# callmeray/PointMVSNet

Hardware: AMD Instinct MI355X
Metric: depth-maps/sec (DTU 640x512, 3 src views, 2 flow iters) (higher is better)
Workload: dtype f32

## Files before the change

include/pointflow_hip.h:

```cpp
#ifndef POINTFLOW_HIP_H_
#define POINTFLOW_HIP_H_

#include <stdint.h>

#ifdef __cplusplus
extern "C" {
#endif

#define PF_OK 0
#define PF_ERR_INVALID_ARG (-1)
#define PF_ERR_UNSUPPORTED (-2)

#define PF_STATUS_BAD_INDEX 1u

#define PF_MAX_VIEWS 8
#define PF_GEMM_TILE 64

#define PF_CAM_KREF_INV 0
#define PF_CAM_RREF_INV 9
#define PF_CAM_TREF 18
#define PF_CAM_MEAN 21
#define PF_CAM_STD 24
#define PF_CAM_VIEWS 27
#define PF_CAM_VIEW_STRIDE 21
// ... 60 lines not shown
typedef struct pf_bn_job {
  const double* partials;
  int32_t T, pcols, col0, C;
  double count, unbias_n;
  const float* gamma;
  const float* beta;
  float* running_mean;
  float* running_var;
  float momentum, eps;
  int32_t G, groups_per_stat;
  float* scale;
  float* shift;
  int32_t ld_affine;
  int32_t rows4;
} pf_bn_job;
int pf_bn_finalize_jobs_f32(const pf_bn_job* jobs, int njobs, void* stream);


int pf_pointwise_gemm_f32(const float* X, int x_point_major, int64_t ldx, const float* Wt, float* Y,
                          int64_t ldy, int G, int Ng, int K, int Nc, int Nc_store, const float* in_scale,
                          const float* in_shift, const pf_bn_job* in_bn, int groups_per_stat, double* col_partials,
                          void* stream);

int pf_edge_stats_f32(const float* LE, int64_t ldle, int C, const int64_t* idx, int k, int G, int Ng,
                      double* partials, const uint8_t* codes, int lat_ks, int lat_h, int lat_w, void* stream);


int pf_edge_apply_f32(const float* LE, int64_t ldle, int C, const int64_t* idx, int k, int G, int Ng,
                      const float* scale, const float* shift, int ld_affine, int groups_per_stat,
                      int concat, float* Y, int64_t ldy, const uint8_t* codes, int lat_ks, int lat_h, int lat_w,
                      void* stream);

int pf_edge_backward_reduce_f32(const float* LE, int64_t ldle, int C, const int64_t* idx, int k, int G, int Ng,
                                const float* grad_y, int64_t ldg, const float* scale, const float* shift,
                                const float* mean, const float* invstd, int ld_affine, int groups_per_stat,
                                int concat, double* partials, void* stream);
int pf_edge_backward_apply_f32(const float* LE, int64_t ldle, int C, const int64_t* idx, int k, int G, int Ng,
                               const float* grad_y, int64_t ldg, const float* scale, const float* shift,
                               const float* mean, const float* invstd, const float* c1, const float* c2,
                               int ld_affine, int groups_per_stat, int concat, float* grad_le,
                               const uint32_t* inv_order, const uint32_t* inv_start, void* stream);

int pf_edge_backward_sums_f32(const float* LE, int64_t ldle, int C, const int64_t* idx, int k, int G, int Ng,
                              const float* grad_y, int64_t ldg, const float* scale, const float* shift,
                              const float* mean, const float* invstd, int ld_affine, int groups_per_stat, int concat,
                              double* partials, float* grad_le, float* grad_acc, int64_t ld_acc, int plane,
                              void* stream);
int pf_edge_backward_finish_f32(const float* LE, int64_t ldle, int C, int k, int G, int Ng, const float* grad_y,
                                int64_t ldg, const float* scale, const float* shift, const float* mean,
                                const float* invstd, const float* c1, const float* c2, int ld_affine,
                                int groups_per_stat, int concat, float* grad_le, const uint32_t* inv_order,
                                const uint32_t* inv_start, int plane, void* stream);

int pf_edge_backward_coeffs_f32(const double* partials, int G, int T, int cbn, int C, int concat, int groups_per_stat,
// ... 234 lines not shown
```

pointmvsnet_amd/_lib.py:

```python
import ctypes
import os

import torch

_HERE = os.path.dirname(os.path.abspath(__file__))
LIB_PATH = os.environ.get("PF_LIB_PATH") or os.path.join(_HERE, "libpointflow_hip.so")

_vp, _i, _i64, _f, _d = ctypes.c_void_p, ctypes.c_int, ctypes.c_int64, ctypes.c_float, ctypes.c_double



class BnJob(ctypes.Structure):
    _fields_ = [("partials", _vp), ("T", ctypes.c_int32), ("pcols", ctypes.c_int32), ("col0", ctypes.c_int32),
                ("C", ctypes.c_int32), ("count", _d), ("unbias_n", _d), ("gamma", _vp), ("beta", _vp),
                ("running_mean", _vp), ("running_var", _vp), ("momentum", _f), ("eps", _f),
                ("G", ctypes.c_int32), ("groups_per_stat", ctypes.c_int32), ("scale", _vp), ("shift", _vp),
                ("ld_affine", ctypes.c_int32), ("rows4", ctypes.c_int32)]


class WgradItem(ctypes.Structure):
    _fields_ = [("gr", _vp), ("x", _vp)] + [(n, _i64) for n in ("N", "Cg", "Cx", "Do", "Ho", "Wo", "Di", "Hi", "Wi")] + \
               [(n, ctypes.c_int32) for n in ("KD", "KH", "KW", "stride", "pd", "ph", "pw", "x_samples_per_stat")] + \
               [("x_scale", _vp), ("x_shift", _vp), ("workspace", _vp), ("workspace_bytes", _i64)] + \
               [(n, _i64) for n in ("rows_P", "ldg", "ldx", "x_rows_per_stat")]
# ... 34 lines not shown
    "pf_deconv3d_k3s2_f32": ([_vp, _vp, _vp, _vp, _i64, _i64, _i64, _i64, _i64, _i64, _vp, _vp, ctypes.POINTER(BnJob), _i,
                              _vp, _vp], _i),
    "pf_conv3d_bottom_supported": ([_i64, _i64, _i], _i),
    "pf_conv3d_bottom_blocks": ([_i64, _i64, _i64, _i], _i),
    "pf_conv3d_bottom_f32": ([_vp, _vp, _vp, _i64, _i64, _i64, _i64, _i64, _i64, _i, _vp, _vp, ctypes.POINTER(BnJob), _i,
                              _vp, _vp], _i),
    "pf_deconv3d_bottom_supported": ([_i64, _i64], _i),
    "pf_deconv3d_bottom_blocks": ([_i64, _i64, _i64], _i),
    "pf_deconv3d_bottom_f32": ([_vp, _vp, _vp, _i64, _i64, _i64, _i64, _i64, _i64, _vp, _vp, ctypes.POINTER(BnJob), _i,
                                _vp, _vp], _i),
    "pf_conv2d_wide_supported": ([_i64, _i64, _i, _i], _i),
    "pf_conv2d_wide_blocks": ([_i64, _i64, _i64, _i], _i),
    "pf_conv2d_wide_f32": ([_vp, _vp, _vp, _i64, _i64, _i64, _i64, _i64, _i, _i, _vp, _vp, ctypes.POINTER(BnJob), _i,
                            _vp, _i, _vp], _i),
    "pf_conv2d_wide_sets_f32": ([_vp, _i, _vp, _i64, _i, _vp, _i64, _i64, _i64, _i64, _i64, _i, _i, _vp, _vp,
                                 ctypes.POINTER(BnJob), _i, _vp, _i, _vp], _i),
    "pf_norm_blocks": ([_i64], _i),
    "pf_channel_stats_f32": ([_vp, _i64, _i64, _i64, _vp, _vp], _i),
    "pf_channel_affine_f32": ([_vp, _vp, _vp, _vp, _i64, _i64, _i64, _i, _i, _vp], _i),
    "pf_channel_bn_apply_f32": ([_vp, _vp, _vp, _i, _i64, _i64, _i64, _i, _d, _vp, _vp, _vp, _vp, _f, _f, _i, _vp, _vp], _i),
    "pf_channel_bn_apply2_f32": ([_vp, _vp, _i, _vp, _vp, _vp, _vp, _f, _f, _vp, _vp, _i, _vp, _vp, _vp, _vp, _f, _f, _vp,
                                  _i64, _i64, _i64, _i, _d, _vp], _i),
    "pf_channel_bn_fused_f32": ([_vp, _vp, _i64, _i64, _i64, _i, _vp, _vp, _vp, _vp, _f, _f, _i, _vp, _vp, _i, _vp], _i),
    "pf_edge_stats_f32": ([_vp, _i64, _i, _vp, _i, _i, _i, _vp, _vp, _i, _i, _i, _vp], _i),
    "pf_edge_backward_reduce_f32": ([_vp, _i64, _i, _vp, _i, _i, _i, _vp, _i64, _vp, _vp, _vp, _vp, _i, _i, _i, _vp, _vp], _i),
    "pf_edge_backward_apply_f32": ([_vp, _i64, _i, _vp, _i, _i, _i, _vp, _i64, _vp, _vp, _vp, _vp, _vp, _vp, _i, _i, _i,
                                    _vp, _vp, _vp, _vp], _i),
    "pf_edge_backward_sums_f32": ([_vp, _i64, _i, _vp, _i, _i, _i, _vp, _i64, _vp, _vp, _vp, _vp, _i, _i, _i, _vp, _vp, _vp,
                                   _i64, _i, _vp], _i),
    "pf_edge_backward_finish_f32": ([_vp, _i64, _i, _i, _i, _i, _vp, _i64, _vp, _vp, _vp, _vp, _vp, _vp, _i, _i, _i,
                                     _vp, _vp, _vp, _i, _vp], _i),
    "pf_knn_inverse_workspace": ([_i, _i, _i], _i64),
    "pf_knn_inverse": ([_vp, _i, _i, _i, _vp, _vp, _vp, _i64, _vp], _i),
    "pf_bn_finalize_f32": ([_vp, _i, _i, _i, _i, _d, _d, _vp, _vp, _vp, _vp, _f, _f, _i, _i, _vp, _vp, _i, _vp], _i),
    "pf_bn_finalize_jobs_f32": ([ctypes.POINTER(BnJob), _i, _vp], _i),
    "pf_edge_apply_f32": ([_vp, _i64, _i, _vp, _i, _i, _i, _vp, _vp, _i, _i, _i, _vp, _i64, _vp, _i, _i, _i, _vp], _i),
    "pf_flow_head_f32": ([_vp, _i64, _vp, _vp, _i, ctypes.POINTER(BnJob), _vp, _vp, _i, _i, _vp, _i, _i, _i, _vp, _vp,
                          _vp], _i),
    "pf_eval_pack_map_f32": ([_vp, _vp, _i, _i, _i, _vp], _i),
    "pf_eval_flow_prob_f32": ([_vp, _vp, _i, _i, _i, _vp], _i),
    "pf_eval_prob_filter_f32": ([_vp, _vp, _vp, _i, _i, _i, _i, _f, _f, _vp, _i, _vp], _i),
    "pf_fuse_stage_a_f32": ([_vp, _vp, _vp, _vp, _i, _i, _i, _f, _f, _f, _vp, _vp, _vp, _vp, _vp], _i),
    "pf_fuse_mark": ([_vp, _vp, _vp, _vp, _i, _i, _i, _i, _i, _vp], _i),
    "pf_fuse_compact_f32": ([_vp, _vp, _vp, _vp, _i64, _i64, _vp, _vp, _vp], _i),
    "pf_geo_filter_f32": ([_vp, _vp, _vp, _vp, _i, _i, _i, _i, _f, _f, _i, _f, _f, _vp, _vp, _vp, _vp, _vp], _i),
    "pf_cloud_cell_keys_f32": ([_vp, _i64, _f, _f, _f, _f, _i, _i, _i, _vp, _vp], _i),
    "pf_cloud_pack_f32": ([_vp, _vp, _i64, _i, _vp, _vp], _i),
    "pf_cloud_thin_round": ([_vp, _vp, _i64, _i, _i, _i, _f, _vp, _vp, _vp, _vp], _i),
    "pf_cloud_nn_cells_f32": ([_vp, _i64, _vp, _vp, _i64, _f, _f, _f, _f, _i, _i, _i, _i, _f, _vp, _vp, _vp, _vp], _i),
    "pf_cloud_nn_wave_f32": ([_vp, _vp, _i64, _i64, _vp, _vp, _i64, _f, _f, _f, _f, _i, _i, _i, _f, _vp, _vp, _vp], _i),
    "pf_cloud_obs_mask_f32": ([_vp, _i64, _vp, _i, _i, _i, _f, _f, _f, _f, _vp, _vp], _i),
    "pf_cloud_above_plane_f32": ([_vp, _i64, _f, _f, _f, _f, _vp, _vp], _i),
    "pf_preprocess_resize_u8": ([_vp, _i, _i, _i, _vp, _vp, _vp, _vp, _i, _i, _i, _vp, _vp, _vp], _i),
    "pf_preprocess_standardise_f32": ([_vp, _vp, _i, _i, _i, _vp, _vp], _i),
    "pf_scan_filter_supported": ([_i] * 7, _i),
    "pf_scan_filter_f32": ([_vp, _vp, _vp, _i, _i, _vp, _i, _i, _i, _i, _i, _i] + [_vp] * 8 + [_f, _f, _vp, _vp, _vp, _vp, _vp], _i),
    "pf_softargmin_prob_f32": ([_vp, _vp, _vp, _vp, _i64, _i64, _i64, _vp], _i),
    "pf_bn_train_rows_f32": ([_vp, _i, _i, _i, _i, _d, _d, _vp, _vp, _vp, _vp, _f, _f, _i, _i, _vp, _i, _i, _i, _vp], _i),
    "pf_bn_bwd_reduce_f32": ([_vp, _vp, _vp, _i64, _i64, _i64, _i, _i, _vp, _vp], _i),
# ... 176 lines not shown
```

pointmvsnet_amd/csrc/edgeconv.hip:

```cpp
#include <stdlib.h>

#include "pf_common.h"
#include "pf_bn_resolve.h"

namespace {

typedef float f32x16 __attribute__((ext_vector_type(16)));

constexpr int TILE = PF_GEMM_TILE;

constexpr int GT = 128;
constexpr int LDA = GT + 2;

template <bool POINT_MAJOR, int NT>
__global__ __launch_bounds__(256, 2) void pointwise_gemm_kernel(
    const float* __restrict__ X, int64_t ldx, const float* __restrict__ Wt, float* __restrict__ Y, int64_t ldy,
    int Ng, int K, int Nc_store, const float* __restrict__ in_scale, const float* __restrict__ in_shift,
    int groups_per_stat, double* __restrict__ partials, int T) {
  constexpr int NC = NT * 32;
  constexpr int KC = NT == 4 ? 16 : 32;
  constexpr int NA = KC * GT / 256;
  constexpr int NW = KC * NC / 256;
  __shared__ __attribute__((aligned(16))) float As[2][KC][LDA];
  __shared__ __attribute__((aligned(16))) float Ws[2][KC][NC];
// ... 378 lines not shown
      const int pd = c / k2, rem = c - pd * k2, ph = rem / lat.ks, pw = rem - ph * lat.ks;
      off = (pd - hk) * lat.H * lat.W + (ph - hk) * lat.W + (pw - hk);
    }
    lut[c] = off;
  }
  __syncthreads();
}

template <int C>
__device__ __forceinline__ void gather_rows_codes(const float* __restrict__ LE, int64_t ldle,
                                                  const uint8_t* __restrict__ cp, const int* lut, int64_t gbase, int n,
                                                  int Ng, int q, float4 (&e)[16]) {
  const uint4 cw = *reinterpret_cast<const uint4*>(cp);
  const unsigned w[4] = {cw.x, cw.y, cw.z, cw.w};
#pragma unroll
  for (int j = 0; j < 16; ++j) {
    const int code = (int)((w[j >> 2] >> (8 * (j & 3))) & 255u);
    int i = n + lut[code];
    i = i < 0 ? 0 : (i > Ng - 1 ? Ng - 1 : i);
    e[j] = ld4(LE + (gbase + i) * ldle + C + 4 * q);
  }
}

template <int C, int K>
__global__ __launch_bounds__(256) void edge_stats_kernel(const float* __restrict__ LE, int64_t ldle,
                                                         const int64_t* __restrict__ idx, int k, int Ng,
                                                         double* __restrict__ partials, int T,
                                                         unsigned* __restrict__ status,
                                                         const uint8_t* __restrict__ codes, Lattice lat) {
  constexpr int Q = C / 4;
  constexpr int PPB = 256 / Q;
  __shared__ double red[256 * 8];
  __shared__ int lut[256];
  if (K == 16 && codes != nullptr) build_code_lut(lut, lat);
  const int tid = threadIdx.x;
  const int q = tid % Q, pl = tid / Q;
  const int g = blockIdx.y, tb = blockIdx.x;
  const int tiles = (Ng + TILE - 1) / TILE;
  const int64_t gbase = (int64_t)g * Ng;
  double ds[4] = {0, 0, 0, 0}, dq[4] = {0, 0, 0, 0};
  bool bad = false;
  const int tile0 = xcd_tile(tb, lat);
  for (int tile = tile0; tile < tiles; tile += T) {
    const int n0 = tile * TILE;
    for (int p = pl; p < TILE; p += PPB) {
      const int n = n0 + p;
      if (n >= Ng) break;
      const int64_t row = gbase + n;
      const float4 l = ld4(LE + row * ldle + 4 * q);
      const int64_t* ip = idx + row * k;
      float4 s = {0, 0, 0, 0}, s2 = {0, 0, 0, 0};
      if constexpr (K > 0) {
        float4 e[K > 0 ? K : 1];
        if constexpr (K == 16) {
          if (codes != nullptr) gather_rows_codes<C>(LE, ldle, codes + row * 16, lut, gbase, n, Ng, q, e);
          else gather_rows<C, 16>(LE, ldle, ip, gbase, Ng, q, e, bad);
// ... 17 lines not shown
          const float dx = e.x - l.x, dy = e.y - l.y, dz = e.z - l.z, dw = e.w - l.w;
          s.x += dx; s.y += dy; s.z += dz; s.w += dw;
          s2.x += dx * dx; s2.y += dy * dy; s2.z += dz * dz; s2.w += dw * dw;
        }
      }
      ds[0] += (double)s.x; ds[1] += (double)s.y; ds[2] += (double)s.z; ds[3] += (double)s.w;
      dq[0] += (double)s2.x; dq[1] += (double)s2.y; dq[2] += (double)s2.z; dq[3] += (double)s2.w;
    }
  }
  if (bad) atomicOr(status, PF_STATUS_BAD_INDEX);
#pragma unroll
  for (int c = 0; c < 4; ++c) {
    red[tid * 8 + c] = ds[c];
    red[tid * 8 + 4 + c] = dq[c];
  }
  __syncthreads();
  if (tid < 2 * C) {
    const int qq = tid / 8, comp = tid % 8;
    double acc = 0.0;
    for (int s = 0; s < PPB; ++s) acc += red[(s * Q + qq) * 8 + comp];
    double* o = partials + (((int64_t)g * T + tile0) * C + 4 * qq + (comp & 3)) * 2 + (comp >> 2);
    *o = acc;
  }
}

template <int C, int K>
__global__ __launch_bounds__(256) void edge_apply_kernel(const float* __restrict__ LE, int64_t ldle,
                                                         const int64_t* __restrict__ idx, int k, int Ng,
                                                         const float* __restrict__ scale,
                                                         const float* __restrict__ shift, int ld_affine,
                                                         int groups_per_stat, int concat, float* __restrict__ Y,
                                                         int64_t ldy, int T, const uint8_t* __restrict__ codes,
                                                         Lattice lat) {
  constexpr int Q = C / 4;
  constexpr int PPB = 256 / Q;
  __shared__ int lut[256];
  if (K == 16 && codes != nullptr) build_code_lut(lut, lat);
  const int tid = threadIdx.x;
  const int q = tid % Q, pl = tid / Q;
  const int g = blockIdx.y, tb = blockIdx.x;
  const int tiles = (Ng + TILE - 1) / TILE;
  const int64_t gbase = (int64_t)g * Ng;
  const int64_t so = (int64_t)(g / groups_per_stat) * ld_affine;
  const int doff = concat ? C : 0;
  const float4 dsc = ld4(scale + so + doff + 4 * q), dsh = ld4(shift + so + doff + 4 * q);
  float4 csc = {0, 0, 0, 0}, csh = {0, 0, 0, 0};
  if (concat) {
    csc = ld4(scale + so + 4 * q);
    csh = ld4(shift + so + 4 * q);
  }
  const float kf = (float)k;
  bool bad = false;
  for (int tile = xcd_tile(tb, lat); tile < tiles; tile += T) {
    const int n0 = tile * TILE;
    for (int p = pl; p < TILE; p += PPB) {
      const int n = n0 + p;
      if (n >= Ng) break;
      const int64_t row = gbase + n;
      const float4 l = ld4(LE + row * ldle + 4 * q);
      const int64_t* ip = idx + row * k;
      float4 a = {0, 0, 0, 0};
      if constexpr (K > 0) {
        float4 e[K > 0 ? K : 1];
        if constexpr (K == 16) {
          if (codes != nullptr) gather_rows_codes<C>(LE, ldle, codes + row * 16, lut, gbase, n, Ng, q, e);
          else gather_rows<C, 16>(LE, ldle, ip, gbase, Ng, q, e, bad);
        } else {
          gather_rows<C, (K > 0 ? K : 2)>(LE, ldle, ip, gbase, Ng, q, e, bad);
        }
#pragma unroll
        for (int j = 0; j < K; ++j) {
          a.x += fmaxf(fmaf(e[j].x - l.x, dsc.x, dsh.x), 0.0f);
          a.y += fmaxf(fmaf(e[j].y - l.y, dsc.y, dsh.y), 0.0f);
          a.z += fmaxf(fmaf(e[j].z - l.z, dsc.z, dsh.z), 0.0f);
          a.w += fmaxf(fmaf(e[j].w - l.w, dsc.w, dsh.w), 0.0f);
        }
      } else {
        for (int j = 0; j < k; ++j) {
          int64_t i = ip[j];
          i = i < 0 ? 0 : (i >= Ng ? Ng - 1 : i);
          const float4 e = ld4(LE + (gbase + i) * ldle + C + 4 * q);
          a.x += fmaxf(fmaf(e.x - l.x, dsc.x, dsh.x), 0.0f);
          a.y += fmaxf(fmaf(e.y - l.y, dsc.y, dsh.y), 0.0f);
          a.z += fmaxf(fmaf(e.z - l.z, dsc.z, dsh.z), 0.0f);
          a.w += fmaxf(fmaf(e.w - l.w, dsc.w, dsh.w), 0.0f);
        }
      }
      float4 yd = {a.x / kf, a.y / kf, a.z / kf, a.w / kf};
      float* yo = Y + row * ldy + 4 * q;
      if (concat) {
        float4 yc = {fmaxf(fmaf(l.x, csc.x, csh.x), 0.0f), fmaxf(fmaf(l.y, csc.y, csh.y), 0.0f),
                     fmaxf(fmaf(l.z, csc.z, csh.z), 0.0f), fmaxf(fmaf(l.w, csc.w, csh.w), 0.0f)};
        *reinterpret_cast<float4*>(yo) = yc;
        *reinterpret_cast<float4*>(yo + C) = yd;
      } else {
        *reinterpret_cast<float4*>(yo) = yd;
      }
    }
  }
  (void)bad;
}

struct EdgeBwdAffine {
  const float* scale;
  const float* shift;
  const float* mean;
  const float* invstd;
  const float* c1;
  const float* c2;
  int ld, groups_per_stat, concat;
};

template <int C, int K, bool SUMS>
__global__ __launch_bounds__(256) void edge_bwd_reduce_kernel(const float* __restrict__ LE, int64_t ldle,
                                                              const int64_t* __restrict__ idx, int k, int Ng,
                                                              const float* __restrict__ Gy, int64_t ldg,
                                                              EdgeBwdAffine A, double* __restrict__ partials, int T,
                                                              unsigned* __restrict__ status, float* __restrict__ sums,
                                                              float* __restrict__ gacc, int64_t lda, int band) {
// ... 668 lines not shown
  if (codes == nullptr) {
    PF_REQUIRE(idx != nullptr);
    if (lat_ks == 0 && lat_h >= 1 && lat_w >= 1 && (int64_t)lat_h * lat_w > 1 && Ng % ((int64_t)lat_h * lat_w) == 0) {
      lat.H = lat_h;
      lat.W = lat_w;
    }
    return PF_OK;
  }
  PF_REQUIRE(k == 16 && (lat_ks == 3 || lat_ks == 5) && lat_h >= 1 && lat_w >= 1);
  PF_REQUIRE(Ng % (lat_h * lat_w) == 0);
  lat.ks = lat_ks;
  lat.H = lat_h;
  lat.W = lat_w;
  return PF_OK;
}

static int xcd_band(int64_t plane, int unit, int64_t Ng, int64_t blocks) {
  static const bool on = !(getenv("PF_EDGE_XCD") && atoi(getenv("PF_EDGE_XCD")) == 0);
  if (!on || plane <= 1 || plane % unit != 0 || (plane / unit) % 8 != 0 || Ng % plane != 0 || blocks != Ng / unit) return 0;
  return (int)(plane / unit / 8);
}
static void lattice_band(Lattice& lat, int Ng, int T) { lat.band = xcd_band((int64_t)lat.H * lat.W, TILE, Ng, T); }

int pf_edge_stats_f32(const float* LE, int64_t ldle, int C, const int64_t* idx, int k, int G, int Ng,
                      double* partials, const uint8_t* codes, int lat_ks, int lat_h, int lat_w, void* stream) {
  PF_REQUIRE(G >= 0 && Ng >= 0 && k >= 1 && ldle >= 2 * (int64_t)C && (ldle % 4) == 0 && G <= 65535);
  if (C != 32 && C != 64 && C != 128) return PF_ERR_UNSUPPORTED;
  if (G == 0 || Ng == 0) return PF_OK;
  PF_REQUIRE(LE && partials);
  Lattice lat;
  {
    const int rc = check_lattice(idx, codes, k, Ng, lat_ks, lat_h, lat_w, lat);
    if (rc != PF_OK) return rc;
  }
  unsigned* status = pf_status_ptr();
  PF_REQUIRE(status != nullptr);
  const int T = pf_stat_blocks(G, Ng);
  lattice_band(lat, Ng, T);
  dim3 grid((unsigned)T, (unsigned)G);
  hipStream_t s = (hipStream_t)stream;
#define PF_ES(CV, KV) hipLaunchKernelGGL((edge_stats_kernel<CV, KV>), grid, dim3(256), 0, s, LE, ldle, idx, k, Ng, partials, T, status, codes, lat)
  if (k == 16) {
    if (C == 32) PF_ES(32, 16); else if (C == 64) PF_ES(64, 16); else PF_ES(128, 16);
  } else {
    if (C == 32) PF_ES(32, 0); else if (C == 64) PF_ES(64, 0); else PF_ES(128, 0);
  }
#undef PF_ES
  return pf_launch_status();
}

int pf_bn_finalize_jobs_f32(const pf_bn_job* jobs, int njobs, void* stream) {
  PF_REQUIRE(jobs != nullptr && njobs >= 1 && njobs <= kBnJobs);
  BnJobs packed;
  int cmax = 0;
  for (int i = 0; i < njobs; ++i) {
    const pf_bn_job& j = jobs[i];
    PF_REQUIRE(j.T >= 1 && j.pcols >= 1 && j.col0 >= 0 && j.C >= 1 && j.col0 + j.C <= j.pcols && j.count > 0.0);
    PF_REQUIRE(j.G >= 1 && j.groups_per_stat >= 1 && (j.G % j.groups_per_stat) == 0 && j.ld_affine >= j.C);
    PF_REQUIRE(j.partials && j.gamma && j.beta && j.scale && j.shift);
    PF_REQUIRE((j.running_mean == nullptr) == (j.running_var == nullptr));
    packed.j[i] = j;
    cmax = j.C > cmax ? j.C : cmax;
  }
  for (int i = njobs; i < kBnJobs; ++i) packed.j[i] = jobs[0];
// ... 12 lines not shown
  j.T = T;
  j.pcols = pcols;
  j.col0 = col0;
  j.C = C;
  j.count = count;
  j.unbias_n = unbias_n;
  j.gamma = gamma;
  j.beta = beta;
  j.running_mean = running_mean;
  j.running_var = running_var;
  j.momentum = momentum;
  j.eps = eps;
  j.G = G;
  j.groups_per_stat = groups_per_stat;
  j.scale = scale;
  j.shift = shift;
  j.ld_affine = ld_affine;
  j.rows4 = 0;
  return pf_bn_finalize_jobs_f32(&j, 1, stream);
}

int pf_edge_apply_f32(const float* LE, int64_t ldle, int C, const int64_t* idx, int k, int G, int Ng,
                      const float* scale, const float* shift, int ld_affine, int groups_per_stat, int concat,
                      float* Y, int64_t ldy, const uint8_t* codes, int lat_ks, int lat_h, int lat_w, void* stream) {
  PF_REQUIRE(G >= 0 && Ng >= 0 && k >= 1 && ldle >= 2 * (int64_t)C && (ldle % 4) == 0 && G <= 65535);
  PF_REQUIRE(groups_per_stat >= 1 && (ldy % 4) == 0 && ldy >= (concat ? 2 : 1) * (int64_t)C);
  PF_REQUIRE((ld_affine % 4) == 0 && ld_affine >= (concat ? 2 : 1) * C);
  if (C != 32 && C != 64 && C != 128) return PF_ERR_UNSUPPORTED;
  if (G == 0 || Ng == 0) return PF_OK;
  PF_REQUIRE(LE && scale && shift && Y);
  Lattice lat;
  {
    const int rc = check_lattice(idx, codes, k, Ng, lat_ks, lat_h, lat_w, lat);
    if (rc != PF_OK) return rc;
  }
  const int T = pf_stat_blocks(G, Ng);
  lattice_band(lat, Ng, T);
  dim3 grid((unsigned)T, (unsigned)G);
  hipStream_t s = (hipStream_t)stream;
#define PF_EA(CV, KV)                                                                                         \
  hipLaunchKernelGGL((edge_apply_kernel<CV, KV>), grid, dim3(256), 0, s, LE, ldle, idx, k, Ng, scale, shift, \
                     ld_affine, groups_per_stat, concat, Y, ldy, T, codes, lat)
  if (k == 16) {
    if (C == 32) PF_EA(32, 16); else if (C == 64) PF_EA(64, 16); else PF_EA(128, 16);
  } else {
    if (C == 32) PF_EA(32, 0); else if (C == 64) PF_EA(64, 0); else PF_EA(128, 0);
  }
#undef PF_EA
  return pf_launch_status();
}

extern "C++" {
static int edge_backward_reduce(const float* LE, int64_t ldle, int C, const int64_t* idx, int k, int G, int Ng,
                                const float* grad_y, int64_t ldg, const float* scale, const float* shift,
                                const float* mean, const float* invstd, int ld_affine, int groups_per_stat,
                                int concat, double* partials, float* sums, float* gacc, int64_t lda, int plane,
                                void* stream) {
  PF_REQUIRE(G >= 0 && Ng >= 0 && k >= 1 && ldle >= 2 * (int64_t)C && (ldle % 4) == 0 && G <= 65535);
  PF_REQUIRE(gacc == nullptr || (sums != nullptr && (lda % 4) == 0 && lda >= (concat ? 2 : 1) * (int64_t)C));
  PF_REQUIRE(groups_per_stat >= 1 && (ldg % 4) == 0 && ldg >= (concat ? 2 : 1) * (int64_t)C);
  PF_REQUIRE((ld_affine % 4) == 0 && ld_affine >= (concat ? 2 : 1) * C);
  if (C != 32 && C != 64) return PF_ERR_UNSUPPORTED;
  if (G == 0 || Ng == 0) return PF_OK;
  PF_REQUIRE(LE && idx && grad_y && scale && shift && mean && invstd && partials);
  unsigned* status = pf_status_ptr();
// ... 154 lines not shown
```

pointmvsnet_amd/pointflow.py:

```python
import contextlib
import ctypes

import torch

from . import _lib
from .utils.torch_utils import knn_lattice

_F32 = torch.float32


def hip_inference(x, module):
    if not (torch.is_tensor(x) and x.is_cuda and x.dtype == _F32):
        return False
    if not torch.is_grad_enabled():
        return True
    return not (x.requires_grad or any(p.requires_grad for p in module.parameters()))


_LIBRARY_WARNED = set()


def warn_library_fallback(what, conv):
    key = (what, type(conv).__name__, conv.in_channels, conv.out_channels, tuple(conv.kernel_size), tuple(conv.stride))
    if key in _LIBRARY_WARNED:
# ... 811 lines not shown

def batch_norm_act2_(x1, bn1, partials1, x2, bn2, partials2, samples_per_stat):
    N, C = x1.shape[:2]
    S = x1[0, 0].numel()
    if x2.shape != x1.shape or not (x1.is_contiguous() and x2.is_contiguous()):
        raise RuntimeError("batch_norm_act2_: the two tensors must be contiguous and of one shape")
    for bn in (bn1, bn2):
        if bn.momentum is None:
            raise NotImplementedError("cumulative-average BatchNorm momentum is not supported")
    def side(bn):
        track = bn.track_running_stats and bn.running_mean is not None
        return (_lib.ptr(bn.weight.detach()), _lib.ptr(bn.bias.detach()), _lib.ptr(bn.running_mean if track else None),
                _lib.ptr(bn.running_var if track else None), float(bn.momentum), float(bn.eps))
    a, b = side(bn1), side(bn2)
    _lib.call("pf_channel_bn_apply2_f32", _lib.ptr(x1), _lib.ptr(partials1), int(partials1.shape[1]), *a,
              _lib.ptr(x2), _lib.ptr(partials2), int(partials2.shape[1]), *b, _lib.ptr(x1), N, C, S,
              int(samples_per_stat), float(samples_per_stat) * S, _lib.stream(), algo_bytes=12.0 * N * C * S)
    G = N // samples_per_stat
    bump_counter(bn1, G)
    bump_counter(bn2, G)
    return x1


def edge_conv_fused(X, point_major, ldx, K, G, Ng, idx, conv1_w, conv2_w, bn, concat, Y, ldy,
                    groups_per_stat=1, join=None, codes=None, lattice=None, keep=None):
    C = conv1_w.shape[0]
    k = idx.shape[-1] if idx is not None else int(codes.shape[-1])
    lat = tuple(int(v) for v in lattice) if lattice is not None else (0, 1, 1)
    if codes is None:
        lat = (0, lat[1], lat[2])
    if keep is not None:
        keep["plane"] = lat[1] * lat[2] if lat[1] * lat[2] > 1 else 0
    dev = Y.device
    S = G // groups_per_stat
    training = bn.training or not bn.track_running_stats
    Wt, _ = pack_weight_t(conv1_w, conv2_w)
    LE = torch.empty((G * Ng, 2 * C), dtype=_F32, device=dev)
    cbn = 2 * C if concat else C
    scale = torch.empty((S, cbn), dtype=_F32, device=dev)
    shift = torch.empty((S, cbn), dtype=_F32, device=dev)
    n_pairs = float(groups_per_stat) * Ng * k
    part_l = pointwise_gemm(X, point_major, ldx, Wt, LE, 2 * C, G, Ng, K, 2 * C, groups_per_stat=groups_per_stat,
                            want_stats=(concat and training))
    if join is not None:
        torch.cuda.current_stream().wait_stream(join)
    rows4 = None
    if training:
        T = stat_blocks(G, Ng)
        part_d = stat_rows(G, T, C, dev)
        _lib.call("pf_edge_stats_f32", _lib.ptr(LE), 2 * C, C, _lib.ptr(idx), k, G, Ng, _lib.ptr(part_d),
                  _lib.ptr(codes), lat[0], lat[1], lat[2], _lib.stream(),
                  algo_bytes=float(G) * Ng * (4.0 * C + (1.0 if codes is not None else 8.0) * k + 4.0 * C * k))
        if keep is not None:
            from . import train_ops
            rows4 = torch.empty((4, S, cbn), dtype=_F32, device=dev)

            def job4(partials, count, unbias_n, col, ch0):
                j = bn_job(bn, partials, 0, C, count, unbias_n, G, groups_per_stat, rows4[0][:, col:], rows4[1][:, col:],
                           ch0=ch0)
                j.rows4 = 1
                return j

            if not train_ops.TRAIN_LAZY_BN:
                if concat:
                    train_ops.bn_train_rows(bn, part_l, 0, C, float(groups_per_stat) * Ng, G, groups_per_stat,
                                            unbias_n=n_pairs, rows=rows4, col_out=0, ch0=0, bump=False)
                    train_ops.bn_train_rows(bn, part_d, 0, C, n_pairs, G, groups_per_stat, rows=rows4, col_out=C, ch0=C,
                                            bump=False)
                else:
                    train_ops.bn_train_rows(bn, part_d, 0, C, n_pairs, G, groups_per_stat, rows=rows4, bump=False)
            elif concat:
                bn_finalize_jobs([job4(part_l, float(groups_per_stat) * Ng, n_pairs, 0, 0),
                                  job4(part_d, n_pairs, n_pairs, C, C)])
            else:
                bn_finalize_jobs([job4(part_d, n_pairs, n_pairs, 0, 0)])
            scale, shift = rows4[0], rows4[1]
        elif concat:
            bn_finalize_jobs([
                bn_job(bn, part_l, 0, C, float(groups_per_stat) * Ng, n_pairs, G, groups_per_stat, scale, shift),
                bn_job(bn, part_d, 0, C, n_pairs, n_pairs, G, groups_per_stat, scale[:, C:], shift[:, C:], ch0=C)])
        else:
            bn_affine(bn, part_d, 0, C, n_pairs, n_pairs, G, groups_per_stat, scale, shift, ch0=0)
        bump_counter(bn, S)
    else:
        sc, sh = eval_affine(bn, S, cbn)
        scale.copy_(sc.unsqueeze(0).expand(S, cbn))
        shift.copy_(sh.unsqueeze(0).expand(S, cbn))
    if keep is not None:
        if not training:
            raise RuntimeError("edge_conv_fused(keep=...) needs a train-mode BatchNorm")
        keep.update(LE=LE, scale=rows4[0], shift=rows4[1], mean=rows4[2], invstd=rows4[3])
    _lib.call("pf_edge_apply_f32", _lib.ptr(LE), 2 * C, C, _lib.ptr(idx), k, G, Ng, _lib.ptr(scale),
              _lib.ptr(shift), cbn, groups_per_stat, int(bool(concat)), _lib.ptr(Y), int(ldy), _lib.ptr(codes),
              lat[0], lat[1], lat[2], _lib.stream(),
              algo_bytes=float(G) * Ng * (4.0 * C + (1.0 if codes is not None else 8.0) * k + 4.0 * C * k + 4.0 * cbn))
    return Y


_inverse_cache = _collections.OrderedDict()


def knn_inverse(idx, G, Ng, k):
    key = (idx.data_ptr(), idx._version, str(idx.device), G, Ng, k)
    hit = _inverse_cache.get(key)
    if hit is not None and hit[0]() is idx:
        return hit[1], hit[2]
    dev = idx.device
    order = torch.empty((G * Ng * k,), dtype=torch.int32, device=dev)
    start = torch.empty((G * Ng + 1,), dtype=torch.int32, device=dev)
    nbytes = int(_lib.load().pf_knn_inverse_workspace(int(G), int(Ng), int(k)))
    work = torch.empty((max(nbytes, 1),), dtype=torch.uint8, device=dev)
    _lib.call("pf_knn_inverse", _lib.ptr(idx), int(k), int(G), int(Ng), _lib.ptr(order), _lib.ptr(start), _lib.ptr(work),
              nbytes, _lib.stream(), algo_bytes=8.0 * G * Ng * k * 4)
    try:
        _inverse_cache[key] = (_weakref.ref(idx), order, start)
    except TypeError:
        return order, start
# ... 140 lines not shown

        def _knn():
            out = knn_lattice(xyz.view(G, 3, 5, hs, ws), 5, k, with_codes=use_codes, with_idx=not use_codes)
            return out if use_codes else (out, None)

        if CONCURRENCY >= 2:
            main = torch.cuda.current_stream()
            aux = side_stream(dev, 1)
            aux.wait_stream(main)
            with torch.cuda.stream(aux):
                idx, codes = _knn()
                (codes if use_codes else idx).record_stream(main)
        else:
            idx, codes = _knn()

    widths = []
    for m in edge_convs:
        c = m.conv1.weight.shape[0]
        widths.append(2 * c if m.concat else c)
    ctot = sum(widths)
    edges = torch.empty((G * Ng, ctot), dtype=_F32, device=dev)
    col = 0
    X, pm, ldx, K = feature, bool(point_major), (Cin if point_major else 0), Cin
    for li, (m, wdt) in enumerate(zip(edge_convs, widths)):
        Y = edges[:, col:]
        edge_conv_fused(X, pm, ldx, K, G, Ng, idx, m.conv1.weight, m.conv2.weight, m.bn, m.concat, Y, ctot,
                        join=(aux if li == 0 else None), codes=codes, lattice=lattice)
        X, pm, ldx, K = Y, True, ctot, wdt
        col += wdt

    shared, last = flow_mlp[0], flow_mlp[1]
    X, ldx, K = edges, ctot, ctot
    affine = None
    for layer in shared:
        Wt, cout = pack_weight_t(layer.conv.weight)
        Z = torch.empty((G * Ng, cout), dtype=_F32, device=dev)
        bn = layer.bn
        part = pointwise_gemm(X, True, ldx, Wt, Z, cout, G, Ng, K, cout, in_affine=affine, want_stats=True)
        affine = _bn_affine_from_gemm(bn, part, cout, G, Ng, 1, dev, lazy=True)
        X, ldx, K = Z, cout, cout
    if K != 16 or last.weight.shape[0] != 1:
        raise NotImplementedError("flow head kernel is built for the reference widths (..., 16, 1)")
    depth_out = torch.empty((h, w), dtype=_F32, device=dev)
    flow_prob = torch.empty((5, h, w), dtype=_F32, device=dev)
    w_out = last.weight.detach().reshape(-1).to(_F32).contiguous()
    sc, sh, in_bn = _split_affine(affine)
    _lib.call("pf_flow_head_f32", _lib.ptr(X), ldx, _lib.ptr(sc), _lib.ptr(sh), 16, in_bn,
              _lib.ptr(w_out), _lib.ptr(depth), int(depth.shape[-2]), int(depth.shape[-1]), _lib.ptr(interval), h, w,
              ratio, _lib.ptr(flow_prob), _lib.ptr(depth_out), _lib.stream(),
              algo_bytes=4.0 * G * Ng * 16 + 4.0 * h * w * 7)
# ... 23 lines not shown
```

Before: 1086.

## Fold edge BN finalize into stats and apply kernels via lazy affine jobs

In the edge-conv stats kernel, the last-arriving block of each row group (chosen with an atomic ticket counter) pre-reduces the per-tile partials into a smaller set of combined rows. The edge apply kernel then receives BN jobs and resolves scale and shift in-kernel, instead of relying on a separate BN finalize launch. It overlaps the first point's gather with this resolution. The goal is to remove the finalize kernel launch and its host-side sequencing per edge conv, at the cost of redundant per-block reductions in apply plus ticket and fence synchronization.

```diff
diff --git a/include/pointflow_hip.h b/include/pointflow_hip.h
--- a/include/pointflow_hip.h
+++ b/include/pointflow_hip.h
@@ -106,14 +106,16 @@
                           const float* in_shift, const pf_bn_job* in_bn, int groups_per_stat, double* col_partials,
                           void* stream);
 
+int pf_edge_stat_rows(int G, int Ng, int C, int groups_per_stat);
 int pf_edge_stats_f32(const float* LE, int64_t ldle, int C, const int64_t* idx, int k, int G, int Ng,
-                      double* partials, const uint8_t* codes, int lat_ks, int lat_h, int lat_w, void* stream);
+                      double* partials, const uint8_t* codes, int lat_ks, int lat_h, int lat_w, double* rows,
+                      unsigned* tickets, int groups_per_stat, void* stream);
 
 
 int pf_edge_apply_f32(const float* LE, int64_t ldle, int C, const int64_t* idx, int k, int G, int Ng,
                       const float* scale, const float* shift, int ld_affine, int groups_per_stat,
                       int concat, float* Y, int64_t ldy, const uint8_t* codes, int lat_ks, int lat_h, int lat_w,
-                      void* stream);
+                      const pf_bn_job* in_bn_d, const pf_bn_job* in_bn_c, void* stream);
 
 int pf_edge_backward_reduce_f32(const float* LE, int64_t ldle, int C, const int64_t* idx, int k, int G, int Ng,
                                 const float* grad_y, int64_t ldg, const float* scale, const float* shift,
diff --git a/pointmvsnet_amd/_lib.py b/pointmvsnet_amd/_lib.py
--- a/pointmvsnet_amd/_lib.py
+++ b/pointmvsnet_amd/_lib.py
@@ -80,7 +80,8 @@
     "pf_channel_bn_apply2_f32": ([_vp, _vp, _i, _vp, _vp, _vp, _vp, _f, _f, _vp, _vp, _i, _vp, _vp, _vp, _vp, _f, _f, _vp,
                                   _i64, _i64, _i64, _i, _d, _vp], _i),
     "pf_channel_bn_fused_f32": ([_vp, _vp, _i64, _i64, _i64, _i, _vp, _vp, _vp, _vp, _f, _f, _i, _vp, _vp, _i, _vp], _i),
-    "pf_edge_stats_f32": ([_vp, _i64, _i, _vp, _i, _i, _i, _vp, _vp, _i, _i, _i, _vp], _i),
+    "pf_edge_stat_rows": ([_i, _i, _i, _i], _i),
+    "pf_edge_stats_f32": ([_vp, _i64, _i, _vp, _i, _i, _i, _vp, _vp, _i, _i, _i, _vp, _vp, _i, _vp], _i),
     "pf_edge_backward_reduce_f32": ([_vp, _i64, _i, _vp, _i, _i, _i, _vp, _i64, _vp, _vp, _vp, _vp, _i, _i, _i, _vp, _vp], _i),
     "pf_edge_backward_apply_f32": ([_vp, _i64, _i, _vp, _i, _i, _i, _vp, _i64, _vp, _vp, _vp, _vp, _vp, _vp, _i, _i, _i,
                                     _vp, _vp, _vp, _vp], _i),
@@ -92,7 +93,8 @@
     "pf_knn_inverse": ([_vp, _i, _i, _i, _vp, _vp, _vp, _i64, _vp], _i),
     "pf_bn_finalize_f32": ([_vp, _i, _i, _i, _i, _d, _d, _vp, _vp, _vp, _vp, _f, _f, _i, _i, _vp, _vp, _i, _vp], _i),
     "pf_bn_finalize_jobs_f32": ([ctypes.POINTER(BnJob), _i, _vp], _i),
-    "pf_edge_apply_f32": ([_vp, _i64, _i, _vp, _i, _i, _i, _vp, _vp, _i, _i, _i, _vp, _i64, _vp, _i, _i, _i, _vp], _i),
+    "pf_edge_apply_f32": ([_vp, _i64, _i, _vp, _i, _i, _i, _vp, _vp, _i, _i, _i, _vp, _i64, _vp, _i, _i, _i,
+                           ctypes.POINTER(BnJob), ctypes.POINTER(BnJob), _vp], _i),
     "pf_flow_head_f32": ([_vp, _i64, _vp, _vp, _i, ctypes.POINTER(BnJob), _vp, _vp, _i, _i, _vp, _i, _i, _i, _vp, _vp,
                           _vp], _i),
     "pf_eval_pack_map_f32": ([_vp, _vp, _i, _i, _i, _vp], _i),
diff --git a/pointmvsnet_amd/csrc/edgeconv.hip b/pointmvsnet_amd/csrc/edgeconv.hip
--- a/pointmvsnet_amd/csrc/edgeconv.hip
+++ b/pointmvsnet_amd/csrc/edgeconv.hip
@@ -424,16 +424,24 @@
   }
 }
 
+struct StatRows {
+  double* rows;
+  unsigned* tickets;
+  int R, Tr;
+};
+
 template <int C, int K>
 __global__ __launch_bounds__(256) void edge_stats_kernel(const float* __restrict__ LE, int64_t ldle,
                                                          const int64_t* __restrict__ idx, int k, int Ng,
                                                          double* __restrict__ partials, int T,
                                                          unsigned* __restrict__ status,
-                                                         const uint8_t* __restrict__ codes, Lattice lat) {
+                                                         const uint8_t* __restrict__ codes, Lattice lat,
+                                                         StatRows sr) {
   constexpr int Q = C / 4;
   constexpr int PPB = 256 / Q;
   __shared__ double red[256 * 8];
   __shared__ int lut[256];
+  __shared__ unsigned last_s;
   if (K == 16 && codes != nullptr) build_code_lut(lut, lat);
   const int tid = threadIdx.x;
   const int q = tid % Q, pl = tid / Q;
@@ -497,60 +505,142 @@
     double* o = partials + (((int64_t)g * T + tile0) * C + 4 * qq + (comp & 3)) * 2 + (comp >> 2);
     *o = acc;
   }
-}
-
-template <int C, int K>
+  if (sr.rows == nullptr) return;
+  __threadfence();
+  __syncthreads();
+  const int rg = tile0 / sr.R;
+  const int members = min(sr.R, T - rg * sr.R);
+  if (tid == 0) {
+    unsigned* t = sr.tickets + (int64_t)g * sr.Tr + rg;
+    const bool last = atomicAdd(t, 1u) + 1u == (unsigned)members;
+    if (last) *t = 0u;
+    last_s = last ? 1u : 0u;
+  }
+  __syncthreads();
+  if (last_s == 0u) return;
+  __threadfence();
+  if (tid < 2 * C) {
+    const unsigned long long* src =
+        reinterpret_cast<const unsigned long long*>(partials + ((int64_t)g * T + (int64_t)rg * sr.R) * C * 2) + tid;
+    double acc = 0.0;
+    for (int r0 = 0; r0 < members; r0 += 4) {
+      unsigned long long v[4];
+#pragma unroll
+      for (int u = 0; u < 4; ++u) v[u] = __atomic_load_n(src + (int64_t)min(r0 + u, members - 1) * C * 2, __ATOMIC_RELAXED);
+#pragma unroll
+      for (int u = 0; u < 4; ++u) acc += (r0 + u < members) ? __builtin_bit_cast(double, v[u]) : 0.0;
+    }
+    sr.rows[((int64_t)g * sr.Tr + rg) * C * 2 + tid] = acc;
+  }
+}
+
+template <int C, int K, bool LAZY>
 __global__ __launch_bounds__(256) void edge_apply_kernel(const float* __restrict__ LE, int64_t ldle,
                                                          const int64_t* __restrict__ idx, int k, int Ng,
                                                          const float* __restrict__ scale,
                                                          const float* __restrict__ shift, int ld_affine,
                                                          int groups_per_stat, int concat, float* __restrict__ Y,
                                                          int64_t ldy, int T, const uint8_t* __restrict__ codes,
-                                                         Lattice lat) {
+                                                         Lattice lat, pf_bn_job jd, pf_bn_job jc) {
   constexpr int Q = C / 4;
   constexpr int PPB = 256 / Q;
+  constexpr int KE = K > 0 ? K : 1;
   __shared__ int lut[256];
+  __shared__ __attribute__((aligned(16))) float aff_s[LAZY ? 4 * C : 4];
+  __shared__ double bn_red[LAZY ? 512 : 1];
   if (K == 16 && codes != nullptr) build_code_lut(lut, lat);
   const int tid = threadIdx.x;
   const int q = tid % Q, pl = tid / Q;
   const int g = blockIdx.y, tb = blockIdx.x;
   const int tiles = (Ng + TILE - 1) / TILE;
   const int64_t gbase = (int64_t)g * Ng;
-  const int64_t so = (int64_t)(g / groups_per_stat) * ld_affine;
-  const int doff = concat ? C : 0;
-  const float4 dsc = ld4(scale + so + doff + 4 * q), dsh = ld4(shift + so + doff + 4 * q);
-  float4 csc = {0, 0, 0, 0}, csh = {0, 0, 0, 0};
-  if (concat) {
-    csc = ld4(scale + so + 4 * q);
-    csh = ld4(shift + so + 4 * q);
+  float4 dsc = {0, 0, 0, 0}, dsh = {0, 0, 0, 0}, csc = {0, 0, 0, 0}, csh = {0, 0, 0, 0};
+  if (!LAZY) {
+    const int64_t so = (int64_t)(g / groups_per_stat) * ld_affine;
+    const int doff = concat ? C : 0;
+    dsc = ld4(scale + so + doff + 4 * q);
+    dsh = ld4(shift + so + doff + 4 * q);
+    if (concat) {
+      csc = ld4(scale + so + 4 * q);
+      csh = ld4(shift + so + 4 * q);
+    }
   }
   const float kf = (float)k;
   bool bad = false;
-  for (int tile = xcd_tile(tb, lat); tile < tiles; tile += T) {
+  auto load_point = [&](int n, float4& l, float4 (&e)[KE]) {
+    const int64_t row = gbase + n;
+    l = ld4(LE + row * ldle + 4 * q);
+    const int64_t* ip = idx + row * k;
+    if constexpr (K == 16) {
+      if (codes != nullptr) gather_rows_codes<C>(LE, ldle, codes + row * 16, lut, gbase, n, Ng, q, e);
+      else gather_rows<C, 16>(LE, ldle, ip, gbase, Ng, q, e, bad);
+    } else if constexpr (K > 0) {
+      gather_rows<C, K>(LE, ldle, ip, gbase, Ng, q, e, bad);
+    }
+  };
+  auto store_point = [&](int n, const float4& l, const float4& a) {
+    const int64_t row = gbase + n;
+    float4 yd = {a.x / kf, a.y / kf, a.z / kf, a.w / kf};
+    float* yo = Y + row * ldy + 4 * q;
+    if (concat) {
+      float4 yc = {fmaxf(fmaf(l.x, csc.x, csh.x), 0.0f), fmaxf(fmaf(l.y, csc.y, csh.y), 0.0f),
+                   fmaxf(fmaf(l.z, csc.z, csh.z), 0.0f), fmaxf(fmaf(l.w, csc.w, csh.w), 0.0f)};
+      *reinterpret_cast<float4*>(yo) = yc;
+      *reinterpret_cast<float4*>(yo + C) = yd;
+    } else {
+      *reinterpret_cast<float4*>(yo) = yd;
+    }
+  };
+  auto finish_point = [&](int n, const float4& l, const float4 (&e)[KE]) {
+    float4 a = {0, 0, 0, 0};
+#pragma unroll
+    for (int j = 0; j < K; ++j) {
+      a.x += fmaxf(fmaf(e[j].x - l.x, dsc.x, dsh.x), 0.0f);
+      a.y += fmaxf(fmaf(e[j].y - l.y, dsc.y, dsh.y), 0.0f);
+      a.z += fmaxf(fmaf(e[j].z - l.z, dsc.z, dsh.z), 0.0f);
+      a.w += fmaxf(fmaf(e[j].w - l.w, dsc.w, dsh.w), 0.0f);
+    }
+    store_point(n, l, a);
+  };
+  int tile = xcd_tile(tb, lat);
+  int p = pl;
+  if constexpr (LAZY) {
+    const int n = tile * TILE + p;
+    const bool have = K > 0 && tile < tiles && n < Ng;
+    float4 l, e[KE];
+    if constexpr (K > 0) {
+      if (have) load_point(n, l, e);
+    }
+    const int s = g / groups_per_stat;
+    pf_bn_resolve<256>(jd, s, aff_s, aff_s + C, bn_red);
+    if (concat) pf_bn_resolve<256>(jc, s, aff_s + 2 * C, aff_s + 3 * C, bn_red);
+    dsc = ld4(aff_s + 4 * q);
+    dsh = ld4(aff_s + C + 4 * q);
+    if (concat) {
+      csc = ld4(aff_s + 2 * C + 4 * q);
+      csh = ld4(aff_s + 3 * C + 4 * q);
+    }
+    if constexpr (K > 0) {
+      if (have) {
+        finish_point(n, l, e);
+        p += PPB;
+      }
+    }
+  }
+  for (; tile < tiles; tile += T, p = pl) {
     const int n0 = tile * TILE;
-    for (int p = pl; p < TILE; p += PPB) {
+    for (; p < TILE; p += PPB) {
       const int n = n0 + p;
       if (n >= Ng) break;
-      const int64_t row = gbase + n;
-      const float4 l = ld4(LE + row * ldle + 4 * q);
-      const int64_t* ip = idx + row * k;
-      float4 a = {0, 0, 0, 0};
       if constexpr (K > 0) {
-        float4 e[K > 0 ? K : 1];
-        if constexpr (K == 16) {
-          if (codes != nullptr) gather_rows_codes<C>(LE, ldle, codes + row * 16, lut, gbase, n, Ng, q, e);
-          else gather_rows<C, 16>(LE, ldle, ip, gbase, Ng, q, e, bad);
-        } else {
-          gather_rows<C, (K > 0 ? K : 2)>(LE, ldle, ip, gbase, Ng, q, e, bad);
-        }
-#pragma unroll
-        for (int j = 0; j < K; ++j) {
-          a.x += fmaxf(fmaf(e[j].x - l.x, dsc.x, dsh.x), 0.0f);
-          a.y += fmaxf(fmaf(e[j].y - l.y, dsc.y, dsh.y), 0.0f);
-          a.z += fmaxf(fmaf(e[j].z - l.z, dsc.z, dsh.z), 0.0f);
-          a.w += fmaxf(fmaf(e[j].w - l.w, dsc.w, dsh.w), 0.0f);
-        }
+        float4 l, e[KE];
+        load_point(n, l, e);
+        finish_point(n, l, e);
       } else {
+        const int64_t row = gbase + n;
+        const float4 l = ld4(LE + row * ldle + 4 * q);
+        const int64_t* ip = idx + row * k;
+        float4 a = {0, 0, 0, 0};
         for (int j = 0; j < k; ++j) {
           int64_t i = ip[j];
           i = i < 0 ? 0 : (i >= Ng ? Ng - 1 : i);
@@ -560,16 +650,7 @@
           a.z += fmaxf(fmaf(e.z - l.z, dsc.z, dsh.z), 0.0f);
           a.w += fmaxf(fmaf(e.w - l.w, dsc.w, dsh.w), 0.0f);
         }
-      }
-      float4 yd = {a.x / kf, a.y / kf, a.z / kf, a.w / kf};
-      float* yo = Y + row * ldy + 4 * q;
-      if (concat) {
-        float4 yc = {fmaxf(fmaf(l.x, csc.x, csh.x), 0.0f), fmaxf(fmaf(l.y, csc.y, csh.y), 0.0f),
-                     fmaxf(fmaf(l.z, csc.z, csh.z), 0.0f), fmaxf(fmaf(l.w, csc.w, csh.w), 0.0f)};
-        *reinterpret_cast<float4*>(yo) = yc;
-        *reinterpret_cast<float4*>(yo + C) = yd;
-      } else {
-        *reinterpret_cast<float4*>(yo) = yd;
+        store_point(n, l, a);
       }
     }
   }
@@ -1284,9 +1365,23 @@
 }
 static void lattice_band(Lattice& lat, int Ng, int T) { lat.band = xcd_band((int64_t)lat.H * lat.W, TILE, Ng, T); }
 
+static int edge_rows_per_combined(int T, int C, int groups_per_stat) {
+  int R = 4;
+  while ((int64_t)groups_per_stat * pf_cdiv(T, R) * C > 4096 && R < T) R *= 2;
+  return R;
+}
+
+int pf_edge_stat_rows(int G, int Ng, int C, int groups_per_stat) {
+  if (G <= 0 || Ng <= 0 || C <= 0 || groups_per_stat <= 0) return 0;
+  const int T = pf_stat_blocks(G, Ng);
+  return (int)pf_cdiv(T, edge_rows_per_combined(T, C, groups_per_stat));
+}
+
 int pf_edge_stats_f32(const float* LE, int64_t ldle, int C, const int64_t* idx, int k, int G, int Ng,
-                      double* partials, const uint8_t* codes, int lat_ks, int lat_h, int lat_w, void* stream) {
+                      double* partials, const uint8_t* codes, int lat_ks, int lat_h, int lat_w, double* rows,
+                      unsigned* tickets, int groups_per_stat, void* stream) {
   PF_REQUIRE(G >= 0 && Ng >= 0 && k >= 1 && ldle >= 2 * (int64_t)C && (ldle % 4) == 0 && G <= 65535);
+  PF_REQUIRE((rows == nullptr) == (tickets == nullptr) && (rows == nullptr || groups_per_stat >= 1));
   if (C != 32 && C != 64 && C != 128) return PF_ERR_UNSUPPORTED;
   if (G == 0 || Ng == 0) return PF_OK;
   PF_REQUIRE(LE && partials);
@@ -1301,7 +1396,12 @@
   lattice_band(lat, Ng, T);
   dim3 grid((unsigned)T, (unsigned)G);
   hipStream_t s = (hipStream_t)stream;
-#define PF_ES(CV, KV) hipLaunchKernelGGL((edge_stats_kernel<CV, KV>), grid, dim3(256), 0, s, LE, ldle, idx, k, Ng, partials, T, status, codes, lat)
+  StatRows sr{rows, tickets, 1, T};
+  if (rows != nullptr) {
+    sr.R = edge_rows_per_combined(T, C, groups_per_stat);
+    sr.Tr = (int)pf_cdiv(T, sr.R);
+  }
+#define PF_ES(CV, KV) hipLaunchKernelGGL((edge_stats_kernel<CV, KV>), grid, dim3(256), 0, s, LE, ldle, idx, k, Ng, partials, T, status, codes, lat, sr)
   if (k == 16) {
     if (C == 32) PF_ES(32, 16); else if (C == 64) PF_ES(64, 16); else PF_ES(128, 16);
   } else {
@@ -1360,13 +1460,34 @@
 
 int pf_edge_apply_f32(const float* LE, int64_t ldle, int C, const int64_t* idx, int k, int G, int Ng,
                       const float* scale, const float* shift, int ld_affine, int groups_per_stat, int concat,
-                      float* Y, int64_t ldy, const uint8_t* codes, int lat_ks, int lat_h, int lat_w, void* stream) {
+                      float* Y, int64_t ldy, const uint8_t* codes, int lat_ks, int lat_h, int lat_w,
+                      const pf_bn_job* in_bn_d, const pf_bn_job* in_bn_c, void* stream) {
   PF_REQUIRE(G >= 0 && Ng >= 0 && k >= 1 && ldle >= 2 * (int64_t)C && (ldle % 4) == 0 && G <= 65535);
   PF_REQUIRE(groups_per_stat >= 1 && (ldy % 4) == 0 && ldy >= (concat ? 2 : 1) * (int64_t)C);
-  PF_REQUIRE((ld_affine % 4) == 0 && ld_affine >= (concat ? 2 : 1) * C);
   if (C != 32 && C != 64 && C != 128) return PF_ERR_UNSUPPORTED;
+  if (in_bn_d != nullptr) {
+    PF_REQUIRE(scale == nullptr && shift == nullptr && (in_bn_c != nullptr) == (concat != 0));
+    if (G == 0 || Ng == 0) return PF_OK;
+    PF_REQUIRE(G % groups_per_stat == 0);
+    int rc = pf_bn_in_check(in_bn_d, C, G / groups_per_stat);
+    if (rc == PF_OK && concat) rc = pf_bn_in_check(in_bn_c, C, G / groups_per_stat);
+    if (rc == PF_ERR_UNSUPPORTED) {
+      const pf_bn_job* first = concat ? in_bn_c : in_bn_d;
+      PF_REQUIRE(!concat || (in_bn_d->scale == in_bn_c->scale + C && in_bn_d->shift == in_bn_c->shift + C &&
+                             in_bn_d->ld_affine == in_bn_c->ld_affine));
+      rc = bn_materialize_rows(in_bn_d, (hipStream_t)stream);
+      if (rc == PF_OK && concat) rc = bn_materialize_rows(in_bn_c, (hipStream_t)stream);
+      if (rc != PF_OK) return rc;
+      return pf_edge_apply_f32(LE, ldle, C, idx, k, G, Ng, first->scale, first->shift, first->ld_affine, groups_per_stat,
+                               concat, Y, ldy, codes, lat_ks, lat_h, lat_w, nullptr, nullptr, stream);
+    }
+    if (rc != PF_OK) return rc;
+  } else {
+    PF_REQUIRE(in_bn_c == nullptr);
+    PF_REQUIRE((ld_affine % 4) == 0 && ld_affine >= (concat ? 2 : 1) * C);
+  }
   if (G == 0 || Ng == 0) return PF_OK;
-  PF_REQUIRE(LE && scale && shift && Y);
+  PF_REQUIRE(LE && Y && (in_bn_d != nullptr || (scale && shift)));
   Lattice lat;
   {
     const int rc = check_lattice(idx, codes, k, Ng, lat_ks, lat_h, lat_w, lat);
@@ -1376,9 +1497,16 @@
   lattice_band(lat, Ng, T);
   dim3 grid((unsigned)T, (unsigned)G);
   hipStream_t s = (hipStream_t)stream;
-#define PF_EA(CV, KV)                                                                                         \
-  hipLaunchKernelGGL((edge_apply_kernel<CV, KV>), grid, dim3(256), 0, s, LE, ldle, idx, k, Ng, scale, shift, \
-                     ld_affine, groups_per_stat, concat, Y, ldy, T, codes, lat)
+  const pf_bn_job no_bn = {};
+#define PF_EA(CV, KV)                                                                                                   \
+  do {                                                                                                                  \
+    if (in_bn_d != nullptr)                                                                                             \
+      hipLaunchKernelGGL((edge_apply_kernel<CV, KV, true>), grid, dim3(256), 0, s, LE, ldle, idx, k, Ng, scale, shift,  \
+                         ld_affine, groups_per_stat, concat, Y, ldy, T, codes, lat, *in_bn_d, concat ? *in_bn_c : no_bn); \
+    else                                                                                                                \
+      hipLaunchKernelGGL((edge_apply_kernel<CV, KV, false>), grid, dim3(256), 0, s, LE, ldle, idx, k, Ng, scale, shift, \
+                         ld_affine, groups_per_stat, concat, Y, ldy, T, codes, lat, no_bn, no_bn);                      \
+  } while (0)
   if (k == 16) {
     if (C == 32) PF_EA(32, 16); else if (C == 64) PF_EA(64, 16); else PF_EA(128, 16);
   } else {
diff --git a/pointmvsnet_amd/pointflow.py b/pointmvsnet_amd/pointflow.py
--- a/pointmvsnet_amd/pointflow.py
+++ b/pointmvsnet_amd/pointflow.py
@@ -857,8 +857,17 @@
     return x1
 
 
+def edge_stat_rows(G, Ng, C, groups_per_stat=1):
+    return int(_lib.load().pf_edge_stat_rows(int(G), int(Ng), int(C), int(groups_per_stat)))
+
+
+def edge_stat_tickets(G, Ng, widths, groups_per_stat, dev):
+    n = max(edge_stat_rows(G, Ng, c, groups_per_stat) for c in widths)
+    return torch.zeros((max(G * n, 1),), dtype=torch.int32, device=dev)
+
+
 def edge_conv_fused(X, point_major, ldx, K, G, Ng, idx, conv1_w, conv2_w, bn, concat, Y, ldy,
-                    groups_per_stat=1, join=None, codes=None, lattice=None, keep=None):
+                    groups_per_stat=1, join=None, codes=None, lattice=None, keep=None, tickets=None):
     C = conv1_w.shape[0]
     k = idx.shape[-1] if idx is not None else int(codes.shape[-1])
     lat = tuple(int(v) for v in lattice) if lattice is not None else (0, 1, 1)
@@ -880,13 +889,33 @@
     if join is not None:
         torch.cuda.current_stream().wait_stream(join)
     rows4 = None
+    in_d = in_c = None
     if training:
         T = stat_blocks(G, Ng)
         part_d = stat_rows(G, T, C, dev)
+        rows_d = None
+        if keep is None and LAZY_BN and bn.momentum is not None:
+            Tr = edge_stat_rows(G, Ng, C, groups_per_stat)
+            if groups_per_stat * Tr * C <= LAZY_MAX_ELEMS and (
+                    not concat or groups_per_stat * part_l.shape[1] * C <= LAZY_MAX_ELEMS):
+                rows_d = stat_rows(G, Tr, C, dev)
+                if tickets is None:
+                    tickets = edge_stat_tickets(G, Ng, (C,), groups_per_stat, dev)
+                if tickets.numel() < G * Tr or tickets.dtype != torch.int32:
+                    raise RuntimeError("edge_conv_fused: tickets must hold G * edge_stat_rows() int32 counters")
         _lib.call("pf_edge_stats_f32", _lib.ptr(LE), 2 * C, C, _lib.ptr(idx), k, G, Ng, _lib.ptr(part_d),
-                  _lib.ptr(codes), lat[0], lat[1], lat[2], _lib.stream(),
+                  _lib.ptr(codes), lat[0], lat[1], lat[2], _lib.ptr(rows_d),
+                  _lib.ptr(tickets if rows_d is not None else None), groups_per_stat, _lib.stream(),
                   algo_bytes=float(G) * Ng * (4.0 * C + (1.0 if codes is not None else 8.0) * k + 4.0 * C * k))
-        if keep is not None:
+        if rows_d is not None:
+            doff = C if concat else 0
+            alive = (rows_d, part_l, scale, shift) + _bn_tensors(bn)
+            in_d = LazyAffine(bn_job(bn, rows_d, 0, C, n_pairs, n_pairs, G, groups_per_stat, scale[:, doff:],
+                                     shift[:, doff:], ch0=doff), alive, scale, shift)
+            if concat:
+                in_c = LazyAffine(bn_job(bn, part_l, 0, C, float(groups_per_stat) * Ng, n_pairs, G, groups_per_stat,
+                                         scale, shift), alive, scale, shift)
+        elif keep is not None:
             from . import train_ops
             rows4 = torch.empty((4, S, cbn), dtype=_F32, device=dev)
 
@@ -925,9 +954,12 @@
         if not training:
             raise RuntimeError("edge_conv_fused(keep=...) needs a train-mode BatchNorm")
         keep.update(LE=LE, scale=rows4[0], shift=rows4[1], mean=rows4[2], invstd=rows4[3])
-    _lib.call("pf_edge_apply_f32", _lib.ptr(LE), 2 * C, C, _lib.ptr(idx), k, G, Ng, _lib.ptr(scale),
-              _lib.ptr(shift), cbn, groups_per_stat, int(bool(concat)), _lib.ptr(Y), int(ldy), _lib.ptr(codes),
-              lat[0], lat[1], lat[2], _lib.stream(),
+    jc = in_c.job_ptr() if in_c is not None else None
+    jd = in_d.job_ptr() if in_d is not None else None
+    _lib.call("pf_edge_apply_f32", _lib.ptr(LE), 2 * C, C, _lib.ptr(idx), k, G, Ng,
+              _lib.ptr(None if in_d is not None else scale), _lib.ptr(None if in_d is not None else shift), cbn,
+              groups_per_stat, int(bool(concat)), _lib.ptr(Y), int(ldy), _lib.ptr(codes),
+              lat[0], lat[1], lat[2], jd, jc, _lib.stream(),
               algo_bytes=float(G) * Ng * (4.0 * C + (1.0 if codes is not None else 8.0) * k + 4.0 * C * k + 4.0 * cbn))
     return Y
 
@@ -1114,10 +1146,11 @@
     edges = torch.empty((G * Ng, ctot), dtype=_F32, device=dev)
     col = 0
     X, pm, ldx, K = feature, bool(point_major), (Cin if point_major else 0), Cin
+    tickets = edge_stat_tickets(G, Ng, [m.conv1.weight.shape[0] for m in edge_convs], 1, dev) if LAZY_BN else None
     for li, (m, wdt) in enumerate(zip(edge_convs, widths)):
         Y = edges[:, col:]
         edge_conv_fused(X, pm, ldx, K, G, Ng, idx, m.conv1.weight, m.conv2.weight, m.bn, m.concat, Y, ctot,
-                        join=(aux if li == 0 else None), codes=codes, lattice=lattice)
+                        join=(aux if li == 0 else None), codes=codes, lattice=lattice, tickets=tickets)
         X, pm, ldx, K = Y, True, ctot, wdt
         col += wdt
 
```

New measurement: 554.6. 0.511x the previous value.
